# PolyU-IOR/HPR-LP-C

Hardware: AMD Instinct MI355X
Metric: HPR iterations/sec (FP64) (higher is better)
Workload: dtype f64

## Files before the change

hpr-lp-c_amd/csrc/kernels.hip:

```cpp
#include "kernels.h"
#include "group_table.h"
#include "values_body.h"

#include <algorithm>
#include <array>
#include <cstring>
#include <tuple>
#include <stdexcept>
#include <vector>
#include <cmath>
#include <type_traits>

namespace hprlp {

__device__ __forceinline__ double wave_sum(double v) {
#pragma unroll
    for (int off = 32; off > 0; off >>= 1) v += __shfl_xor(v, off, kWave);
    return v;
}

__device__ __forceinline__ double wave_max(double v) {
#pragma unroll
    for (int off = 32; off > 0; off >>= 1) v = fmax(v, __shfl_xor(v, off, kWave));
    return v;
// ... 199 lines not shown
                int j = rs;
                for (; j + 8 <= re; j += 8) {
#pragma unroll
                    for (int v = 0; v < NV; ++v) {
                        double p[8];
#pragma unroll
                        for (int u = 0; u < 8; ++u) p[u] = lds[wave][v][j + u];
#pragma unroll
                        for (int u = 0; u < 8; ++u) s[v] += p[u];
                    }
                }
                if (j < re) {
#pragma unroll
                    for (int v = 0; v < NV; ++v) {
                        double p[8];
#pragma unroll
                        for (int u = 0; u < 8; ++u) p[u] = lds[wave][v][min(j + u, re - 1)];
#pragma unroll
                        for (int u = 0; u < 8; ++u)
                            if (j + u < re) s[v] += p[u];
                    }
                }
                epi.apply(r0 + lane, rw, s, acc);
            }
        }
    }
    if constexpr (NACC > 0) block_store_partials_at<NACC, kWavesPerBlock, MaxAccs<Epi>::value>(acc, epi.partials, epi.stride, bid);
}

template <class Epi>
__global__ void __launch_bounds__(kThreads) k_spmv_fused(CsrDev A, Epi epi) {
    spmv_fused_body<Epi>(A, epi, blockIdx.x, gridDim.x);
}

__device__ __forceinline__ void lds_barrier() { asm volatile("s_waitcnt lgkmcnt(0)\n\ts_barrier" ::: "memory"); }

__device__ __forceinline__ int step_field(int a0, int a1, int a2, int a3, int r) {
    const int q = r >> 6;
    const int v = q == 0 ? a0 : (q == 1 ? a1 : (q == 2 ? a2 : a3));
    return __builtin_amdgcn_readlane(v, r & 63);
}

#ifndef HPRLP_PB_PHASE_STAMPS
#define HPRLP_PB_PHASE_STAMPS 0
#endif
#ifndef HPRLP_SWEEP_ED
#define HPRLP_SWEEP_ED 2
#define HPRLP_SWEEP_TD 1
#endif
#ifndef HPRLP_EPI_NT
#define HPRLP_EPI_NT 2
#endif

template <int ED, int TD, bool REP, bool STAMP = false, bool LOGTERM = false, int TC = kTileCols>
__device__ __forceinline__ void tiled_sweep(const TiledDev &t, int s0, int nst, int first, int count, const double *__restrict__ vec,
                                            int ncols, double *acc, double *ytile, int tid, unsigned long long *stamp = nullptr) {
    constexpr int NT = kTileThreads, R = kTileRows, K = kTileChunk;
    constexpr int TPT = TC / NT;
    static_assert(TC == kTileCols || TC == kTileColsNarrow, "tile width");
    typedef double d2_t __attribute__((ext_vector_type(2)));
    const int lane = tid & 63;
    auto sidx = [&](int i) { i = min(i, count - 1) + first; return s0 + (i < nst ? i : i - nst); };
    int seg = 0, lim = 0;
    int tc0 = 0, tc1 = 0, tc2 = 0, tc3 = 0, tb0 = 0, tb1 = 0, tb2 = 0, tb3 = 0, te0 = 0, te1 = 0, te2 = 0, te3 = 0;
    auto getstep = [&](int k, int &col0, int &eb, int &ee) {
        const int r = min(k, lim - 1) - seg;
        col0 = step_field(tc0, tc1, tc2, tc3, r);
        eb = step_field(tb0, tb1, tb2, tb3, r);
        ee = step_field(te0, te1, te2, te3, r);
    };
    struct Ent {
        d2_t va, vb;
        uint32_t i0, i1, i2;
    };
    typedef uint32_t u3_t __attribute__((ext_vector_type(3), aligned(4)));
    auto issue_entries = [&](Ent &E, int k) {
        int col0, eb, ee_;
        getstep(k, col0, eb, ee_);
        const int e = eb + K * tid;
        const int ee = (e < ee_) ? e : eb;
        E.va = __builtin_nontemporal_load(reinterpret_cast<const d2_t *>(t.tval + ee));
        E.vb = __builtin_nontemporal_load(reinterpret_cast<const d2_t *>(t.tval + ee) + 1);
        const u3_t w = __builtin_nontemporal_load(reinterpret_cast<const u3_t *>(t.tidx3 + (ee / K) * 3));
        E.i0 = w.x;
        E.i1 = w.y;
        E.i2 = w.z;
    };
    typedef double d2u_t __attribute__((ext_vector_type(2), aligned(8)));
    auto issue_tile = [&](double (&tl)[TPT], int k) {
        int col0, eb, ee_;
        getstep(k, col0, eb, ee_);
        static_assert(TPT % 2 == 0, "tile loads come in pairs");
#pragma unroll
        for (int j = 0; j < TPT / 2; ++j) {
            const int p = col0 + 2 * (tid + j * NT);
            const int q = min(p, ncols - 2);
            d2u_t v = *reinterpret_cast<const d2u_t *>(vec + q);
            if (q != p) v.x = v.y;
            tl[2 * j] = v.x;
            tl[2 * j + 1] = v.y;
        }
    };
    auto store_tile = [&](const double (&tl)[TPT]) {
#pragma unroll
        for (int j = 0; j < TPT / 2; ++j) {
            d2_t v;
            v.x = tl[2 * j];
            v.y = tl[2 * j + 1];
            reinterpret_cast<d2_t *>(ytile)[tid + j * NT] = v;
// ... 30 lines not shown
    auto same_tile = [&](int k) {
        if (k <= seg || k >= lim) return false;
        int c0, c1, eb, ee_;
        getstep(k, c0, eb, ee_);
        getstep(k - 1, c1, eb, ee_);
        return c0 == c1;
    };
    unsigned long long tq[6] = {0, 0, 0, 0, 0, 0}, ph[7] = {0, 0, 0, 0, 0, 0, 0};
    auto step = [&](Ent &E, double (&tl)[TPT], int k) {
        if (STAMP) tq[0] = __builtin_amdgcn_s_memtime();
        lds_barrier();
        if (STAMP) tq[1] = __builtin_amdgcn_s_memtime();
        if (STAMP) {
            store_tile(tl);
            tq[2] = __builtin_amdgcn_s_memtime();
            issue_tile(tl, k + TD);
            tq[3] = __builtin_amdgcn_s_memtime();
            lds_barrier();
            tq[4] = __builtin_amdgcn_s_memtime();
            process(E, k);
            asm volatile("s_waitcnt lgkmcnt(0)" ::: "memory");
            tq[5] = __builtin_amdgcn_s_memtime();
            issue_entries(E, k + ED);
            const unsigned long long t6 = __builtin_amdgcn_s_memtime();
            ph[0] += tq[1] - tq[0];
            ph[1] += tq[2] - tq[1];
            ph[2] += tq[3] - tq[2];
            ph[3] += tq[4] - tq[3];
            ph[4] += tq[5] - tq[4];
            ph[5] += t6 - tq[5];
            ph[6] += 1;
            return;
        }
        if (REP) {
            const bool keep = same_tile(k);
            if (!keep) {
                store_tile(tl);
            }
            if (!same_tile(k + TD)) issue_tile(tl, k + TD);
            if (!keep) lds_barrier();
        } else {
            store_tile(tl);
            issue_tile(tl, k + TD);
            lds_barrier();
        }
        process(E, k);
        issue_entries(E, k + ED);
    };
    for (seg = 0; seg < count; seg += 256) {
        lim = min(seg + 256, count);
        {
            const TileStep q0 = t.steps[sidx(seg + lane)], q1 = t.steps[sidx(seg + 64 + lane)];
            const TileStep q2 = t.steps[sidx(seg + 128 + lane)], q3 = t.steps[sidx(seg + 192 + lane)];
            tc0 = q0.col0; tb0 = q0.e_begin; te0 = q0.e_end;
            tc1 = q1.col0; tb1 = q1.e_begin; te1 = q1.e_end;
            tc2 = q2.col0; tb2 = q2.e_begin; te2 = q2.e_end;
            tc3 = q3.col0; tb3 = q3.e_begin; te3 = q3.e_end;
        }
        Ent E[ED];
        double tl[TD][TPT];
        __builtin_amdgcn_sched_barrier(0);
#pragma unroll
        for (int j = -(ED > TD ? ED : TD); j < 0; ++j) {
            if (j + TD >= 0) {
                issue_tile(tl[(j + TD) % TD], seg + j + TD);
                __builtin_amdgcn_sched_barrier(0);
            }
            if (j + ED >= 0) {
                issue_entries(E[(j + ED) % ED], seg + j + ED);
                __builtin_amdgcn_sched_barrier(0);
            }
        }
        constexpr int U = (ED * TD) % 2 == 0 && ED * TD > 2 ? ED * TD : 2 * ED * TD;
        static_assert(U % ED == 0 && U % TD == 0, "the unrolled body must return every register set to its role");
        bool done = false;
        for (int k = seg; !done;) {
#pragma unroll
            for (int u = 0; u < U; ++u) {
                step(E[u % ED], tl[u % TD], k);
                if (++k >= lim) {
                    done = true;
                    break;
                }
            }
        }
    }
    if (STAMP && tid == 0) {
#pragma unroll
        for (int i = 0; i < 7; ++i) stamp[i] += ph[i];
    }
}

template <int K>
__device__ __forceinline__ void remainder_steps(const TiledDev &t, int smid, int s1, double *acc, double *prod, double *bnd, int tid) {
    constexpr int NT = kTileThreads, NW = kTileThreads / 64;
    static_assert(K == 4 || K == 6 || K == 8, "code loads: one or two 16-byte loads, or two 12-byte loads, per lane");
    if (smid >= s1) return;
    const int wave = tid >> 6, lane = tid & 63;
    double *bnd_val = bnd;
    uint32_t *bnd_row = reinterpret_cast<uint32_t *>(bnd + NW);
    constexpr uint32_t NOROW = 0x10000u;
    double pv[K];
    uint32_t cv[K];
    TileStep st = t.steps[smid];
    auto issue = [&](const TileStep &z) {
        const int last = max(z.e_end - z.e_begin - 1, 0);
#pragma unroll
        for (int k = 0; k < K; ++k) pv[k] = __builtin_nontemporal_load(t.P + z.e_begin + min(tid + k * NT, last));
        const int c0 = min(K * tid, max(last + 1 - K, 0));
        if constexpr (K == 6) {
            typedef uint32_t u3_t __attribute__((ext_vector_type(3), aligned(4)));
            const u3_t w0 = __builtin_nontemporal_load(reinterpret_cast<const u3_t *>(t.rq + z.e_begin + c0));
            const u3_t w1 = __builtin_nontemporal_load(reinterpret_cast<const u3_t *>(t.rq + z.e_begin + c0 + 3));
            cv[0] = w0.x; cv[1] = w0.y; cv[2] = w0.z; cv[3] = w1.x; cv[4] = w1.y; cv[5] = w1.z;
        } else {
            typedef uint32_t u4_t __attribute__((ext_vector_type(4), aligned(4)));
            const u4_t w0 = __builtin_nontemporal_load(reinterpret_cast<const u4_t *>(t.rq + z.e_begin + c0));
            cv[0] = w0.x; cv[1] = w0.y; cv[2] = w0.z; cv[3] = w0.w;
            if constexpr (K == 8) {
                const u4_t w1 = __builtin_nontemporal_load(reinterpret_cast<const u4_t *>(t.rq + z.e_begin + c0 + 4));
                cv[4] = w1.x; cv[5] = w1.y; cv[6] = w1.z; cv[7] = w1.w;
            }
        }
    };
    issue(st);
    for (int s = smid; s < s1; ++s) {
        const int cnt = st.e_end - st.e_begin;
        const TileStep nxt = t.steps[min(s + 1, s1 - 1)];
        lds_barrier();
#pragma unroll
        for (int k = 0; k < K; ++k) {
            const int el = tid + k * NT;
            if (el < cnt) prod[el] = pv[k];
        }
        uint32_t code[K];
        {
            const int shift = K * tid - min(K * tid, max(cnt - K, 0));
#pragma unroll
            for (int u = 0; u < K; ++u) code[u] = cv[u];
            if (shift > 0 && shift < K) {
#pragma unroll
                for (int u = 0; u < K; ++u) {
                    uint32_t c = 0;
#pragma unroll
                    for (int q = 0; q < K; ++q) c = (q == u + shift) ? cv[q] : c;
                    code[u] = c;
                }
            }
        }
        if (s + 1 < s1) issue(nxt);
        lds_barrier();
        const int nv = min(max(cnt - K * tid, 0), K);
        uint32_t row[K];
        double pr[K];
#pragma unroll
        for (int u = 0; u < K; ++u) {
            const bool ok = u < nv;
// ... 21 lines not shown
        const bool open_in = lane > 0 && rf == rl_prev && rf != NOROW;
        double v = run;
        int f = (single && open_in) ? 0 : 1;
#pragma unroll
        for (int off = 1; off < 64; off <<= 1) {
            const double vu = __shfl_up(v, off, 64);
            const int fu = __shfl_up(f, off, 64);
            if (lane >= off && !f) {
                v += vu;
                f |= fu;
            }
        }
        const double v_prev = __shfl_up(v, 1, 64);
        const double carry = open_in ? v_prev : 0.0;
        const int next_open = __shfl_down(static_cast<int>(open_in), 1, 64);
        if (!single) acc[rf] += carry + head;
        const double tail = single ? carry + run : run;
        if (lane == 63) {
            bnd_row[wave] = rl;
            bnd_val[wave] = tail;
        } else if (!next_open && rl != NOROW) {
            acc[rl] += tail;
        }
        lds_barrier();
        if (tid < NW) {
            const uint32_t rw = bnd_row[tid];
            bool last_one = rw != NOROW;
            double tot = 0.0;
#pragma unroll
            for (int w = 0; w < NW; ++w) {
                const bool same = bnd_row[w] == rw;
                if (w <= tid && same) tot += bnd_val[w];
                if (w > tid && same) last_one = false;
            }
            if (last_one) acc[rw] += tot;
        }
        st = nxt;
    }
}

template <class Epi, class = void>
struct StagedLoads : std::false_type {};
template <class Epi>
struct StagedLoads<Epi, std::void_t<decltype(std::declval<const Epi &>().load_code(0))>> : std::true_type {};
template <class T>
__device__ __forceinline__ void needed_here(const T &v) {
    static_assert(sizeof(T) % sizeof(double) == 0 && alignof(T) == alignof(double), "a struct of doubles");
    double d[sizeof(T) / sizeof(double)];
    __builtin_memcpy(d, &v, sizeof(T));
#pragma unroll
    for (unsigned k = 0; k < sizeof(T) / sizeof(double); ++k) asm volatile("" ::"v"(d[k]));
}

template <class Epi, bool PUSH>
__device__ __forceinline__ void epilogue_rows(const Epi &epi, double *acc, double (&racc)[Epi::NACC > 0 ? Epi::NACC : 1], int r0, int nr, int tid) {
    constexpr int NT = kTileThreads, B = 4;
    if constexpr (StagedLoads<Epi>::value) {
        using Raw = decltype(epi.load_a(0));
        using Sel = decltype(epi.load_b(0, 0, 0u));
        auto issue_codes = [&](int b0, unsigned (&cd)[B]) {
#pragma unroll
            for (int u = 0; u < B; ++u) cd[u] = epi.load_code(r0 + min(b0 + tid + u * NT, nr - 1));
            __builtin_amdgcn_sched_barrier(0);
        };
        auto batch = [&](int b0, const unsigned (&cd)[B], unsigned (&cdn)[B]) {
            Raw ra[B];
            Sel rs[B];
            double sv[B][1];
#pragma unroll
            for (int u = 0; u < B; ++u) ra[u] = epi.load_a(r0 + min(b0 + tid + u * NT, nr - 1));
            __builtin_amdgcn_sched_barrier(0);
#pragma unroll
            for (int u = 0; u < B; ++u) rs[u] = epi.load_b(r0 + min(b0 + tid + u * NT, nr - 1), r0, cd[u]);
            __builtin_amdgcn_sched_barrier(0);
            issue_codes(b0 + B * NT, cdn);
#pragma unroll
            for (int u = 0; u < B; ++u) sv[u][0] = acc[min(b0 + tid + u * NT, nr - 1)];
#pragma unroll
            for (int u = 0; u < B; ++u) {
                needed_here(ra[u]);
                needed_here(rs[u]);
                asm volatile("" ::"v"(cdn[u]));
            }
            typename Epi::Row rw[B];
#pragma unroll
            for (int u = 0; u < B; ++u) rw[u] = epi.finish(cd[u], ra[u], rs[u]);
#pragma unroll
            for (int u = 0; u < B; ++u) {
                const int i = b0 + tid + u * NT;
                if (i < nr) {
                    if constexpr (PUSH) acc[i] = epi.apply(r0 + i, rw[u], sv[u], racc);
                    else epi.apply(r0 + i, rw[u], sv[u], racc);
                }
            }
        };
        if (nr <= 0) return;
        unsigned cd0[B], cd1[B];
        __builtin_amdgcn_sched_barrier(0);
        issue_codes(0, cd0);
#pragma unroll
        for (int u = 0; u < B; ++u) asm volatile("" ::"v"(cd0[u]));
        for (int b0 = 0;;) {
            batch(b0, cd0, cd1);
            if ((b0 += B * NT) >= nr) break;
            batch(b0, cd1, cd0);
            if ((b0 += B * NT) >= nr) break;
        }
    } else {
        for (int i0 = tid; i0 < nr; i0 += B * NT) {
            typename Epi::Row rw[B];
            double sv[B][1];
#pragma unroll
            for (int u = 0; u < B; ++u) {
                const int i = min(i0 + u * NT, nr - 1);
                rw[u] = epi.load_row(r0 + i);
                sv[u][0] = acc[i];
            }
#pragma unroll
            for (int u = 0; u < B; ++u) {
                const int i = i0 + u * NT;
                if (i < nr) {
                    if constexpr (PUSH) acc[i] = epi.apply(r0 + i, rw[u], sv[u], racc);
                    else epi.apply(r0 + i, rw[u], sv[u], racc);
                }
            }
        }
    }
}

__device__ __forceinline__ void push_products(const FarPush &f, const double *vals, int pb, int pe, int tid) {
    constexpr int NT = kTileThreads, U = 4;
    if (pb >= pe) return;
    double a4[U];
    int p4[U];
    uint16_t c4[U];
    auto load_batch = [&](int k0) {
#pragma unroll
        for (int u = 0; u < U; ++u) {
            const int z = min(k0 + u * NT, pe - 1);
            a4[u] = __builtin_nontemporal_load(f.val + z);
            p4[u] = __builtin_nontemporal_load(f.pos + z);
            c4[u] = __builtin_nontemporal_load(f.lcol + z);
        }
    };
    int k = pb + tid;
    load_batch(k);
    for (; k < pe; k += U * NT) {
        double prd[U];
        int ps[U];
#pragma unroll
        for (int u = 0; u < U; ++u) {
            prd[u] = a4[u] * vals[c4[u]];
// ... 11 lines not shown
    int lo = 0, hi = nr - 1;
    while (lo < hi) {
        const int mid = (lo + hi + 1) >> 1;
        if (tab_k[mid] <= k) lo = mid;
        else hi = mid - 1;
    }
    return tab_p[lo] + (k - tab_k[lo]);
}

__device__ __forceinline__ void push_products_runs(const FarPush &f, const double *vals, int *tab, int g, int pb, int pe, int tid) {
    constexpr int NT = kTileThreads, U = 4;
    if (pb >= pe) return;
    const int r0 = f.rptr[g], nr = f.rptr[g + 1] - r0;
    int *tab_k = tab, *tab_p = tab + kPbRunTabCap;
    double a4[U];
    uint16_t c4[U];
    auto load_batch = [&](int k0) {
#pragma unroll
        for (int u = 0; u < U; ++u) {
            const int z = min(k0 + u * NT, pe - 1);
            a4[u] = __builtin_nontemporal_load(f.val + z);
            c4[u] = __builtin_nontemporal_load(f.lcol + z);
        }
    };
    int k = pb + tid;
    load_batch(k);
    for (int i = tid; i < nr; i += NT) {
        tab_k[i] = f.rk[r0 + i];
        tab_p[i] = f.rp[r0 + i];
    }
    lds_barrier();
    int ps[U];
#pragma unroll
    for (int u = 0; u < U; ++u) ps[u] = run_position(tab_k, tab_p, nr, min(k + u * NT, pe - 1));
    for (; k < pe; k += U * NT) {
        double prd[U];
        int pc[U];
#pragma unroll
        for (int u = 0; u < U; ++u) {
            prd[u] = a4[u] * vals[c4[u]];
            pc[u] = ps[u];
        }
        const int kn = k + U * NT;
        if (kn < pe) load_batch(kn);
#pragma unroll
        for (int u = 0; u < U; ++u)
            if (k + u * NT < pe) f.P[pc[u]] = prd[u];
        if (kn < pe) {
#pragma unroll
            for (int u = 0; u < U; ++u) ps[u] = run_position(tab_k, tab_p, nr, min(kn + u * NT, pe - 1));
        }
    }
}

template <class Epi, bool REP, bool PUSH = false, bool NARROW = false>
__global__ void __launch_bounds__(kTileThreads, 4) k_tiled_fused(CsrDev A, Epi epi) {
    static_assert(Epi::NV == 1, "the tiled kernel stages one gathered vector");
    constexpr int NT = kTileThreads, RMAX = kTileRows, T = kTileCols;
    constexpr int NACC = Epi::NACC;
    __shared__ double acc[RMAX];
    __shared__ __attribute__((aligned(16))) double ytile[T];
    const TiledDev &t = A.tiled;
    const int tid = threadIdx.x;
    const int R = t.R;
    const int per = t.per, slots = gridDim.x / 8;
    const int slot = blockIdx.x / 8;
    double racc[NACC > 0 ? NACC : 1];
#pragma unroll
    for (int i = 0; i < (NACC > 0 ? NACC : 1); ++i) racc[i] = 0.0;
    epi.begin();
    int wg_round = 0;
    const bool wg_stamp = t.wgtimes && tid == 0 && (t.wg_filter == 0 || (PUSH && NACC == 0));
    if (wg_stamp) t.wgtimes[blockIdx.x * 8] = wall_clock64();
    for (int q = slot; q < per; q += slots) {
        const int sb = (blockIdx.x % 8) * per + q;
        if (sb >= t.nsb) break;
        const double *__restrict__ vec = epi.gv[0];
        lds_barrier();
        const int ncols = A.cols;
        for (int i = tid; i < R; i += NT) acc[i] = 0.0;
        const int s0 = t.sb_ptr[sb], smid = t.sb_mid[sb], s1 = t.sb_ptr[sb + 1];
        if (s0 < smid) tiled_sweep<HPRLP_SWEEP_ED, HPRLP_SWEEP_TD, REP, false, LogTerm<Epi>::value, NARROW ? kTileColsNarrow : kTileCols>(t, s0, smid - s0, t.steps[s0].rot, smid - s0, vec, ncols, acc, ytile, tid);
        remainder_steps<kTileRemK>(t, smid, s1, acc, ytile, ytile + kTileRemCap, tid);
        lds_barrier();
        const int r0 = sb * R;
        const int nr = min(R, A.rows - r0);
        int pb = 0, pe = 0;
        if constexpr (PUSH) {
            pb = epi.push.gptr[sb];
            pe = epi.push.gptr[sb + 1];
        }
        epilogue_rows<Epi, PUSH>(epi, acc, racc, r0, nr, tid);
        if constexpr (PUSH) {
            lds_barrier();
            push_products(epi.push, acc, pb, pe, tid);
        }
        if (wg_stamp && ++wg_round <= 5) t.wgtimes[blockIdx.x * 8 + wg_round] = wall_clock64();
    }
    if (wg_stamp) {
        t.wgtimes[blockIdx.x * 8 + 7] = wall_clock64();
        const unsigned hw = __builtin_amdgcn_s_getreg((31 << 11) | 4), xcc = __builtin_amdgcn_s_getreg((31 << 11) | 20);
        t.wgtimes[blockIdx.x * 8 + 6] = (static_cast<unsigned long long>(xcc & 0xfu) << 32) | hw;
    }
    if constexpr (NACC > 0) {
        __syncthreads();
        block_store_partials_in<NACC, kTileThreads / kWave, MaxAccs<Epi>::value>(racc, epi.partials, epi.stride, reinterpret_cast<double(*)[NACC]>(ytile));
    }
}

template <class Epi, bool PUSH = false>
__global__ void __launch_bounds__(kTileThreads, 4) k_pb_fused(CsrDev A, Epi epi) {
    static_assert(Epi::NV == 1, "one gathered vector");
    constexpr int NT = kTileThreads, K = kPbRemK, CAP = kPbRemCap, NW = kTileThreads / 64;
    constexpr int NACC = Epi::NACC;
    __shared__ double acc[kPbRowsMax];
    __shared__ __attribute__((aligned(16))) double prod[CAP];
    __shared__ double bnd[3 * NW];
    const TiledDev &t = A.tiled;
    const int tid = threadIdx.x;
    const int R = t.R;
    const int per = t.per, slots = gridDim.x / 8;
    const int slot = blockIdx.x / 8;
    double racc[NACC > 0 ? NACC : 1];
#pragma unroll
    for (int i = 0; i < (NACC > 0 ? NACC : 1); ++i) racc[i] = 0.0;
    epi.begin();
#if HPRLP_PB_PHASE_STAMPS
    unsigned long long ph[8] = {0, 0, 0, 0, 0, 0, 0, 0}, tq = wall_clock64(), tk0 = tq;
#define PB_STAMP(i) do { const unsigned long long now_ = wall_clock64(); ph[i] += now_ - tq; tq = now_; } while (0)
#else
#define PB_STAMP(i) do { } while (0)
#endif
    for (int q = slot; q < per; q += slots) {
        const int sb = (blockIdx.x % 8) * per + q;
        if (sb >= t.nsb) break;
        lds_barrier();
        for (int i = tid; i < R; i += NT) acc[i] = 0.0;
        const int smid = t.sb_mid[sb], s1 = t.sb_ptr[sb + 1];
        remainder_steps<K>(t, smid, s1, acc, prod, bnd, tid);
        lds_barrier();
        PB_STAMP(4);
        const int r0 = sb * R;
        const int nr = min(R, A.rows - r0);
        int pb = 0, pe = 0;
        if constexpr (PUSH) {
            pb = epi.push.gptr[sb];
            pe = epi.push.gptr[sb + 1];
        }
        epilogue_rows<Epi, PUSH>(epi, acc, racc, r0, nr, tid);
        PB_STAMP(5);
        if constexpr (PUSH) {
            lds_barrier();
            if (epi.push.rk) push_products_runs(epi.push, acc, reinterpret_cast<int *>(prod), sb, pb, pe, tid);
            else push_products(epi.push, acc, pb, pe, tid);
        }
        PB_STAMP(6);
    }
#if HPRLP_PB_PHASE_STAMPS
    if (t.wgtimes && tid == 0 && PUSH && NACC == 0) {
        ph[7] = wall_clock64() - tk0;
        for (int i = 0; i < 8; ++i) t.wgtimes[blockIdx.x * 8 + i] = ph[i];
    }
#endif
#undef PB_STAMP
    if constexpr (NACC > 0) {
        __syncthreads();
        block_store_partials_in<NACC, kTileThreads / kWave, MaxAccs<Epi>::value>(racc, epi.partials, epi.stride, reinterpret_cast<double(*)[NACC]>(prod));
    }
}

template <bool REP, bool STAMP = false, bool NARROW = false>
__global__ void __launch_bounds__(kTileThreads, 4) k_tiled_part(CsrDev A, const double *__restrict__ vec) {
    constexpr int NT = kTileThreads, RMAX = kTileRows, T = kTileCols;
    __shared__ double acc[RMAX];
    __shared__ __attribute__((aligned(16))) double ytile[T];
    const TiledDev &t = A.tiled;
    const int tid = threadIdx.x;
    const int R = t.R;
    const int per = (t.n_pieces + 7) / 8;
    const int pc = (blockIdx.x % 8) * per + blockIdx.x / 8;
    if (pc >= t.n_pieces) return;
    for (int sg = t.piece_ptr[pc]; sg < t.piece_ptr[pc + 1]; ++sg) {
        const int4 d = t.segs[sg];
        const int sb = d.x;
        lds_barrier();
        for (int i = tid; i < R; i += NT) acc[i] = 0.0;
        const int s0 = t.sb_ptr[sb], smid = t.sb_mid[sb], s1 = t.sb_ptr[sb + 1];
        unsigned long long *st = STAMP ? t.stamps + static_cast<size_t>(pc) * 16 : nullptr;
        unsigned long long c0 = 0, c1 = 0, c2 = 0;
        if (STAMP) c0 = __builtin_amdgcn_s_memtime();
        if (d.z > 0) tiled_sweep<3, 2, REP, STAMP, false, NARROW ? kTileColsNarrow : kTileCols>(t, s0, smid - s0, d.y, d.z, vec, A.cols, acc, ytile, tid, st);
        if (STAMP) c1 = __builtin_amdgcn_s_memtime();
        if (d.w) remainder_steps<kTileRemK>(t, smid, s1, acc, ytile, ytile + kTileRemCap, tid);
        lds_barrier();
        if (STAMP) c2 = __builtin_amdgcn_s_memtime();
        double *out = t.parts + static_cast<size_t>(sg) * R;
        for (int i = tid; i < R; i += NT) out[i] = acc[i];
        if (STAMP && tid == 0) {
            st[8] += c1 - c0;
            st[9] += c2 - c1;
            st[10] += __builtin_amdgcn_s_memtime() - c2;
        }
// ... 2502 lines not shown
```

hpr-lp-c_amd/csrc/tiled.cpp:

```cpp
#include "tiled.h"
#include "env.h"

#include <algorithm>
#include <cstdlib>
#include <cstring>
#include <string>
#include <thread>
#include <type_traits>

namespace hprlp {

namespace {

struct Local {
    std::vector<int> sb_steps, sb_mid;
    std::vector<TileStep> steps;
    std::vector<char> step_is_rem;
    std::vector<uint32_t> tidx;
    std::vector<int> tperm, rcol, rperm;
    std::vector<uint16_t> rrow;
    long dense = 0, pad = 0;
};

void build_range(int rows, int cols, const int *rp, const int *ci, int sb0, int sb1, Local *L, int R, int T, int rem_cap) {
// ... 292 lines not shown
    rcol.alloc_zero(h.n_rem + 8);
    rperm.alloc(h.n_rem + 8);
    rrow.alloc_zero(h.n_rem + 8);
    size_t to = 0, ro = 0;
    for (const TiledHost::Piece &pc : h.pieces) {
        if (!pc.tidx.empty()) {
            HIP_CHECK(hipMemcpy(tidx.p + to, pc.tidx.data(), pc.tidx.size() * sizeof(uint32_t), hipMemcpyHostToDevice));
            HIP_CHECK(hipMemcpy(tperm.p + to, pc.tperm.data(), pc.tperm.size() * sizeof(int), hipMemcpyHostToDevice));
        }
        if (!pc.rcol.empty()) {
            HIP_CHECK(hipMemcpy(rcol.p + ro, pc.rcol.data(), pc.rcol.size() * sizeof(int), hipMemcpyHostToDevice));
            HIP_CHECK(hipMemcpy(rperm.p + ro, pc.rperm.data(), pc.rperm.size() * sizeof(int), hipMemcpyHostToDevice));
            HIP_CHECK(hipMemcpy(rrow.p + ro, pc.rrow.data(), pc.rrow.size() * sizeof(uint16_t), hipMemcpyHostToDevice));
        }
        to += pc.tidx.size();
        ro += pc.rcol.size();
    }
    view.valid = true;
    view.R = R;
    view.T = T;
    view.rem_cap = rem_cap;
    view.nsb = nsb;
    view.sb_ptr = sb_ptr.p;
    view.sb_mid = sb_mid.p;
    view.steps = steps.p;
    view.tval = tval.p;
    pack_indices(nullptr);
    view.tidx3 = tidx3.p;
    finish_schedule(nullptr);
}

void DeviceTiled::compare_with(const TiledHost &h) const {
    auto fail = [](const std::string &what) { throw std::runtime_error("tiling check: " + what); };
    if (n_tile != static_cast<long>(h.n_tile)) fail("tile entries " + std::to_string(n_tile) + " vs " + std::to_string(h.n_tile));
    if (n_rem != static_cast<long>(h.n_rem)) fail("remainder entries " + std::to_string(n_rem) + " vs " + std::to_string(h.n_rem));
    if (dense_entries != h.dense_entries || padding != h.padding) fail("dense / padding totals");
    auto same = [&](const char *name, const auto &dbuf, const auto &host) {
        using T = typename std::decay<decltype(host[0])>::type;
        std::vector<T> dev(host.size());
        if (!host.empty()) HIP_CHECK(hipMemcpy(dev.data(), dbuf.p, host.size() * sizeof(T), hipMemcpyDeviceToHost));
        for (size_t i = 0; i < host.size(); ++i)
            if (std::memcmp(&dev[i], &host[i], sizeof(T)) != 0) fail(std::string(name) + " differs at " + std::to_string(i));
    };
    same("sb_ptr", sb_ptr, h.sb_ptr);
    same("sb_mid", sb_mid, h.sb_mid);
    if (static_cast<size_t>(n_steps) != h.steps.size()) fail("step count");
    {
        std::vector<TileStep> dev(h.steps.size());
        if (!dev.empty()) HIP_CHECK(hipMemcpy(dev.data(), steps.p, dev.size() * sizeof(TileStep), hipMemcpyDeviceToHost));
        for (size_t i = 0; i < dev.size(); ++i)
            if (dev[i].col0 != h.steps[i].col0 || dev[i].e_begin != h.steps[i].e_begin || dev[i].e_end != h.steps[i].e_end)
                fail("steps differ at " + std::to_string(i));
    }
    std::vector<uint32_t> a_tidx;
    std::vector<int> a_tperm, a_rcol, a_rperm;
    std::vector<uint16_t> a_rrow;
    for (const TiledHost::Piece &pc : h.pieces) {
        a_tidx.insert(a_tidx.end(), pc.tidx.begin(), pc.tidx.end());
        a_tperm.insert(a_tperm.end(), pc.tperm.begin(), pc.tperm.end());
        a_rcol.insert(a_rcol.end(), pc.rcol.begin(), pc.rcol.end());
        a_rperm.insert(a_rperm.end(), pc.rperm.begin(), pc.rperm.end());
        a_rrow.insert(a_rrow.end(), pc.rrow.begin(), pc.rrow.end());
    }
    {
        std::vector<uint32_t> packed(a_tidx.size() / 4 * 3);
        for (size_t c = 0; c < a_tidx.size() / 4; ++c) {
            const uint32_t e0 = a_tidx[4 * c], e1 = a_tidx[4 * c + 1], e2 = a_tidx[4 * c + 2], e3 = a_tidx[4 * c + 3];
            packed[3 * c] = e0 | (e1 << 24);
            packed[3 * c + 1] = (e1 >> 8) | (e2 << 16);
            packed[3 * c + 2] = (e2 >> 16) | (e3 << 8);
        }
        same("tidx3", tidx3, packed);
    }
    same("tperm", tperm, a_tperm);
    same("rcol", rcol, a_rcol);
    same("rperm", rperm, a_rperm);
    same("rrow", rrow, a_rrow);
}

}
```

hpr-lp-c_amd/csrc/tiled.h:

```cpp
#pragma once

#include <hip/hip_runtime.h>

#include <cstdint>
#include <vector>

#include "common.h"

namespace hprlp {

constexpr int kTileThreads = 512;
constexpr int kTileRows = 8192;
constexpr int kTileCols = 2048;
constexpr int kTileColsNarrow = 1024;
constexpr int kTileChunk = 4;
constexpr int kTileStepCap = kTileThreads * kTileChunk;
constexpr int kTileRemK = 4;
constexpr int kTileRemCap = (kTileThreads - 4) * kTileRemK;
constexpr int kTileRemRun = 16;
#ifndef HPRLP_PB_REM_K
#define HPRLP_PB_REM_K 8
#endif
constexpr int kPbRemK = HPRLP_PB_REM_K;
constexpr int kPbRemCap = kTileThreads * kPbRemK;
// ... 43 lines not shown
        return 0;
    }
};

#ifndef HPRLP_TILE_LAYERS
#define HPRLP_TILE_LAYERS 4
#endif
#ifndef HPRLP_TILE_LAYER_MIN
#define HPRLP_TILE_LAYER_MIN 1024
#endif
constexpr int kTileLayers = HPRLP_TILE_LAYERS;
constexpr int kTileLayerMin = HPRLP_TILE_LAYER_MIN;

constexpr int kTileResidentPerCu = 2;
constexpr int kFarGroup = kTileRows;
constexpr int kFarThreads = 512;
constexpr long kFarWorkMin = 32768;
constexpr long kFarWorkOverMean = 4;

struct TileStep {
    int col0;
    int e_begin;
    int e_end;
    int rot;
};

struct TiledDev {
    bool valid = false;
    int R = kTileRows;
    int rem_cap = kTileRemCap;
    int T = kTileCols;
    int G = kTileRows;
    int nsb = 0;
    int per = 0;
    int grid = 0;
    bool repeats = false;
    int n_pieces = 0;
    const int *piece_ptr = nullptr;
    const int4 *segs = nullptr;
    const int *slot_ptr = nullptr;
    double *parts = nullptr;
    const int4 *side_blk = nullptr;
    int side_nblk = 0;
    const int4 *side_long = nullptr;
    int side_nlong = 0;
    double *side_partial = nullptr;
    const int *side_rows = nullptr;
    double *base = nullptr;
    unsigned long long *stamps = nullptr;
    unsigned long long *wgtimes = nullptr;
    int wg_filter = 0;
    const int *sb_ptr = nullptr;
    const int *sb_mid = nullptr;
    const TileStep *steps = nullptr;
    const double *tval = nullptr;
    const uint32_t *tidx3 = nullptr;
    double *P = nullptr;
    const uint32_t *rq = nullptr;
    int n_groups = 0;
    const int *f_gptr = nullptr;
    const double *f_val = nullptr;
    const int *f_pos = nullptr;
    const uint16_t *f_lcol = nullptr;
    const int *f_rptr = nullptr;
    const int *f_rk = nullptr;
    const int *f_rp = nullptr;
    int f_maxruns = 0;
    const int4 *f_work = nullptr;
    int n_work = 0;
};

struct TiledHost {
    std::vector<int> sb_ptr, sb_mid;
    std::vector<TileStep> steps;
    struct Piece {
        std::vector<uint32_t> tidx;
        std::vector<int> tperm;
        std::vector<int> rcol, rperm;
        std::vector<uint16_t> rrow;
    };
    std::vector<Piece> pieces;
    size_t n_tile = 0, n_rem = 0;
    long dense_entries = 0;
    long padding = 0;
};

bool build_tiled(int rows, int cols, const int *rowptr, const int *col, TiledHost *out, int min_rows,
                 double min_dense_fraction, int R = kTileRows, int T = kTileCols, int rem_cap = kTileRemCap);

void tiled_host_check(int rows, int cols, const int *rp, const int *ci, int R, int T, double min_dense, long out[6]);

void compact_without_rows(long nnz, int rows, const int *rp_dev, const int *rp_c_dev, const int *col_dev, int *col_c, int *map_c, hipStream_t s);

struct DeviceTiled {
    DBuf<int> sb_ptr, sb_mid, tperm, rperm, rcol;
    DBuf<TileStep> steps;
    DBuf<uint32_t> tidx;
    DBuf<uint32_t> tidx3;
    DBuf<uint16_t> rrow;
    DBuf<double> tval;
    DBuf<double> P, f_val;
    DBuf<uint32_t> rq;
    DBuf<int> f_gptr, f_pos, f_perm;
    DBuf<int> f_rptr, f_rk, f_rp;
    DBuf<int4> f_work;
    DBuf<uint16_t> f_lcol;
    TiledDev view;
    long n_tile = 0, n_rem = 0;
    double rem_top_share = 0.0;
    long dense_entries = 0, padding = 0;
    int n_steps = 0;
    void upload(const TiledHost &h, int R = kTileRows, int T = kTileCols, int rem_cap = kTileRemCap);
    void pack_indices(hipStream_t s);
    void build_far(int cols, hipStream_t s, int G = kTileRows);
    void finish_schedule(hipStream_t s);
    int rot_period = 0;
    DBuf<double> parts;
    DBuf<int> piece_ptr, slot_ptr;
    DBuf<unsigned long long> stamps;
    void dump_stamps() const;
    DBuf<unsigned long long> wgtimes;
    DBuf<int4> side_blk, side_long;
    DBuf<int> side_rows;
    DBuf<double> side_partial, base;
    void set_side(int rows, const int *rowptr_host, const std::vector<int> &long_rows);
    void compose_perms(const int *map_dev, hipStream_t s);
    void dump_wgtimes() const;
    DBuf<int4> segs;
    bool build_on_device(int rows, int cols, long nnz, const int *rowptr, const int *col, int min_rows,
                         double min_dense_fraction, hipStream_t s, int R = kTileRows, int T = kTileCols, int rem_cap = kTileRemCap);
    void compare_with(const TiledHost &h) const;
};

void launch_tiled_refresh(const DeviceTiled &t, const double *csr_val, hipStream_t s);
void launch_tiled_refresh_log(const DeviceTiled &t, const double *csr_val, double *tval_log, double *fval_log, hipStream_t s);

}
```

hpr-lp-c_amd/csrc/tiled_build.hip:

```cpp
#include <algorithm>
#include <functional>
#include <cstdlib>
#include <hipcub/hipcub.hpp>

#include <vector>

#include "common.h"
#include "env.h"
#include "kernels.h"
#include "tiled.h"

namespace hprlp {

namespace {

constexpr int K = kTileChunk;
constexpr int kRowBits = kTileRowBits;

__device__ __forceinline__ int row_of_entry(const int *__restrict__ rowptr, int rows, int k) {
    int lo = 0, hi = rows;
    while (hi - lo > 1) {
        const int mid = lo + ((hi - lo) >> 1);
        if (rowptr[mid] <= k) lo = mid;
        else hi = mid;
// ... 285 lines not shown

__global__ void __launch_bounds__(kThreads) k_pack_codes(long nchunk, const uint32_t *__restrict__ code, uint32_t *__restrict__ packed) {
    const long c = static_cast<long>(blockIdx.x) * kThreads + threadIdx.x;
    if (c >= nchunk) return;
    const uint32_t e0 = code[4 * c], e1 = code[4 * c + 1], e2 = code[4 * c + 2], e3 = code[4 * c + 3];
    packed[3 * c] = e0 | (e1 << 24);
    packed[3 * c + 1] = (e1 >> 8) | (e2 << 16);
    packed[3 * c + 2] = (e2 >> 16) | (e3 << 8);
}

}

void DeviceTiled::pack_indices(hipStream_t s) {
    const long nchunk = n_tile / K;
    tidx3.alloc_zero(static_cast<size_t>(nchunk) * 3 + 8);
    if (nchunk > 0) hipLaunchKernelGGL(k_pack_codes, dim3(grid_for(nchunk)), dim3(kThreads), 0, s, nchunk, tidx.p, tidx3.p);
    HIP_CHECK(hipStreamSynchronize(s));
    tidx.release();
}

namespace {

__global__ void __launch_bounds__(kThreads) k_window_widths(int nsb, int T, const int *__restrict__ sb_ptr, const int *__restrict__ sb_mid,
                                                           const TileStep *__restrict__ steps, unsigned long long *__restrict__ out) {
    const int sb = blockIdx.x * kThreads + threadIdx.x;
    if (sb >= nsb) return;
    const int s0 = sb_ptr[sb], smid = sb_mid[sb];
    if (s0 >= smid) return;
    const int w = (steps[smid - 1].col0 - steps[s0].col0) / T + 1;
    atomicAdd(out, static_cast<unsigned long long>(w));
    atomicAdd(out + 1, 1ull);
    int rep = 0;
    for (int s = s0 + 1; s < smid; ++s) rep += steps[s].col0 == steps[s - 1].col0;
    if (rep) atomicAdd(out + 2, static_cast<unsigned long long>(rep));
}

__global__ void __launch_bounds__(kThreads) k_rotation(int nsb, int period, int T, const int *__restrict__ sb_ptr, const int *__restrict__ sb_mid,
                                                      TileStep *__restrict__ steps) {
    const int sb = blockIdx.x * kThreads + threadIdx.x;
    if (sb >= nsb) return;
    const int s0 = sb_ptr[sb], smid = sb_mid[sb];
    if (s0 >= smid) return;
    const int nst = smid - s0;
    const int w0 = steps[s0].col0 / T;
    const long target = static_cast<long>((w0 + period - 1) / period) * period * T;
    int lo = 0, hi = nst;
    while (lo < hi) {
        const int mid = (lo + hi) >> 1;
        if (steps[s0 + mid].col0 < target) lo = mid + 1; else hi = mid;
    }
    steps[s0].rot = lo < nst ? lo : 0;
}

}

void DeviceTiled::finish_schedule(hipStream_t s) {
    const int nsb = view.nsb;
    int dev = 0, cus = 256;
    HIP_CHECK(hipGetDevice(&dev));
    HIP_CHECK(hipDeviceGetAttribute(&cus, hipDeviceAttributeMultiprocessorCount, dev));
    const int resident = std::max(1, cus / 8) * kTileResidentPerCu;
    view.per = (nsb + 7) / 8;
    view.grid = 8 * std::min(view.per, resident);
    view.n_pieces = 0;
    int want = (nsb > 0 && nsb <= resident * 8) ? resident * 8 : 0;
    if (view.R < kTileRows && nsb >= cus) want = 0;
    if (view.rem_cap != kTileRemCap) want = 0;
    if (const char *e = env_get("HPRLP_TILE_PIECES")) want = std::max(0, std::atoi(e));
    if (want > 0 && nsb > 0) {
        std::vector<int> h_ptr(static_cast<size_t>(nsb) + 1), h_mid(static_cast<size_t>(nsb));
        sb_ptr.download(h_ptr.data(), h_ptr.size());
        sb_mid.download(h_mid.data(), h_mid.size());
        long total = 0;
        for (int sb = 0; sb < nsb; ++sb) total += h_ptr[sb + 1] - h_ptr[sb];
        const int np = static_cast<int>(std::max<long>(1, std::min<long>(want, std::max<long>(total, 1))));
        std::vector<int4> h_segs;
        std::vector<int> h_piece(static_cast<size_t>(np) + 1, 0), h_slot(static_cast<size_t>(nsb) + 1, 0);
        long g = 0;
        std::vector<std::vector<int4>> by_piece(static_cast<size_t>(np));
        for (int sb = 0; sb < nsb; ++sb) {
            const int nst = h_mid[sb] - h_ptr[sb];
            h_slot[sb] = 0;
            if (nst == 0) {
                const int pc = static_cast<int>(total > 0 ? std::min<long>(np - 1, g * np / total) : 0);
                by_piece[pc].push_back(make_int4(sb, 0, 0, 1));
                g += h_ptr[sb + 1] - h_mid[sb];
                continue;
            }
            int done = 0;
            while (done < nst) {
                const int pc = static_cast<int>(std::min<long>(np - 1, (g + done) * np / total));
                const long nxt = pc + 1 >= np ? total : ((static_cast<long>(pc) + 1) * total + np - 1) / np;
                const int cnt = static_cast<int>(std::min<long>(nst - done, std::max<long>(1, nxt - (g + done))));
                by_piece[pc].push_back(make_int4(sb, done, cnt, done + cnt == nst ? 1 : 0));
                done += cnt;
            }
            g += h_ptr[sb + 1] - h_ptr[sb];
        }
        for (int pc = 0; pc < np; ++pc) {
            h_piece[pc] = static_cast<int>(h_segs.size());
            for (const int4 &sg : by_piece[pc]) h_segs.push_back(sg);
        }
        h_piece[np] = static_cast<int>(h_segs.size());
        {
            size_t i = 0;
            for (int sb = 0; sb < nsb; ++sb) {
                h_slot[sb] = static_cast<int>(i);
                while (i < h_segs.size() && h_segs[i].x == sb) ++i;
            }
            h_slot[nsb] = static_cast<int>(i);
            if (i != h_segs.size()) throw std::runtime_error("piece schedule: segments out of super-block order");
        }
        piece_ptr.alloc(h_piece.size()); piece_ptr.upload(h_piece.data(), h_piece.size());
        slot_ptr.alloc(h_slot.size()); slot_ptr.upload(h_slot.data(), h_slot.size());
        segs.alloc(h_segs.size()); segs.upload(h_segs.data(), h_segs.size());
        parts.alloc_zero(h_segs.size() * static_cast<size_t>(view.R));
        view.n_pieces = np;
        view.piece_ptr = piece_ptr.p;
        view.slot_ptr = slot_ptr.p;
        view.segs = segs.p;
        view.parts = parts.p;
        if (const char *e = env_get("HPRLP_TILE_STAMPS"); e && e[0] == '1' && !view.repeats) {
            stamps.alloc_zero(static_cast<size_t>(np) * 16);
            view.stamps = stamps.p;
        }
    }
    if (const char *e = env_get("HPRLP_WG_TIMES"); e && (e[0] == '1' || e[0] == '2') && view.grid > 0) {
        wgtimes.alloc_zero(static_cast<size_t>(view.grid) * 8);
        view.wgtimes = wgtimes.p;
        view.wg_filter = e[0] == '2';
    }
    rot_period = 0;
    if (nsb <= 0 || n_steps <= 0) return;
    {
        DBuf<unsigned long long> acc(3);
        HIP_CHECK(hipMemsetAsync(acc.p, 0, 3 * sizeof(unsigned long long), s));
        hipLaunchKernelGGL(k_window_widths, dim3(grid_for(nsb)), dim3(kThreads), 0, s, nsb, view.T, sb_ptr.p, sb_mid.p, steps.p, acc.p);
        unsigned long long h[3] = {0, 0, 0};
        HIP_CHECK(hipMemcpyAsync(h, acc.p, sizeof(h), hipMemcpyDeviceToHost, s));
        HIP_CHECK(hipStreamSynchronize(s));
        if (h[1] > 0) rot_period = static_cast<int>((h[0] + h[1] - 1) / h[1]);
        view.repeats = h[2] > 0;
    }
    if (const char *e = env_get("HPRLP_TILE_ROT")) rot_period = std::atoi(e);
    if (rot_period > 0) hipLaunchKernelGGL(k_rotation, dim3(grid_for(nsb)), dim3(kThreads), 0, s, nsb, rot_period, view.T, sb_ptr.p, sb_mid.p, steps.p);
    HIP_CHECK(hipStreamSynchronize(s));
}

bool DeviceTiled::build_on_device(int rows, int cols, long nnz, const int *rowptr, const int *col, int min_rows,
                                  double min_dense_fraction, hipStream_t s, int R, int T, int rem_cap) {
    if (rem_cap != kTileRemCap && rem_cap != kPbRemCap) throw std::runtime_error("tiled build: unsupported remainder step size");
    if (rem_cap == kPbRemCap && R > kPbRowsMax) throw std::runtime_error("tiled build: the all-remainder form takes super-blocks of at most 4096 rows");
    if (rows < min_rows || rows <= 0 || cols <= 0 || nnz <= 0 || nnz >= 2000000000L) return false;
    if (R < 64 || R > kTileRows || R % 64 != 0) throw std::runtime_error("tiled build: unsupported super-block height");
    if (T != kTileCols && T != kTileColsNarrow) throw std::runtime_error("tiled build: unsupported tile width");
    const int nsb = (rows + R - 1) / R;
    const int ntile = (cols + T - 1) / T;
    int tile_bits = 1;
    while ((1 << tile_bits) < ntile) ++tile_bits;
    int sb_bits = 1;
    while ((1 << sb_bits) < nsb) ++sb_bits;
    const int key_bits = sb_bits + tile_bits + kRowBits;

    DBuf<unsigned long long> key_in(static_cast<size_t>(nnz)), skey(static_cast<size_t>(nnz));
    DBuf<int> idx_in(static_cast<size_t>(nnz)), sperm(static_cast<size_t>(nnz));
    hipLaunchKernelGGL(k_make_keys, dim3(grid_for(nnz)), dim3(kThreads), 0, s, nnz, rows, tile_bits, R, T, rowptr, col, key_in.p, idx_in.p);
    size_t tmp_bytes = 0;
    HIP_CHECK(hipcub::DeviceRadixSort::SortPairs(nullptr, tmp_bytes, key_in.p, skey.p, idx_in.p, sperm.p, static_cast<int>(nnz), kRowBits,
                                                 key_bits, s));
    {
        DBuf<char> tmp(tmp_bytes + 16);
        HIP_CHECK(hipcub::DeviceRadixSort::SortPairs(tmp.p, tmp_bytes, key_in.p, skey.p, idx_in.p, sperm.p, static_cast<int>(nnz), kRowBits,
                                                     key_bits, s));
        HIP_CHECK(hipStreamSynchronize(s));
    }
    key_in.release();
    idx_in.release();

    DBuf<int> head(static_cast<size_t>(nnz)), run_incl(static_cast<size_t>(nnz));
    hipLaunchKernelGGL(k_run_heads, dim3(grid_for(nnz)), dim3(kThreads), 0, s, nnz, skey.p, head.p);
    HIP_CHECK(hipcub::DeviceScan::InclusiveSum(nullptr, tmp_bytes, head.p, run_incl.p, static_cast<int>(nnz), s));
    {
        DBuf<char> tmp(tmp_bytes + 16);
        HIP_CHECK(hipcub::DeviceScan::InclusiveSum(tmp.p, tmp_bytes, head.p, run_incl.p, static_cast<int>(nnz), s));
        HIP_CHECK(hipStreamSynchronize(s));
    }
    int nruns = 0;
    HIP_CHECK(hipMemcpy(&nruns, run_incl.p + (nnz - 1), sizeof(int), hipMemcpyDeviceToHost));
    DBuf<int> run_start(static_cast<size_t>(nruns) + 1);
    hipLaunchKernelGGL(k_run_starts, dim3(grid_for(nnz)), dim3(kThreads), 0, s, nnz, head.p, run_incl.p, run_start.p);
    {
        const int end = static_cast<int>(nnz);
        HIP_CHECK(hipMemcpyAsync(run_start.p + nruns, &end, sizeof(int), hipMemcpyHostToDevice, s));
        HIP_CHECK(hipStreamSynchronize(s));
    }
    head.release();
    run_incl.release();

// ... 531 lines not shown
```

Before: 790.0.

## Prefetch next super-block descriptor and epilogue codes to hide load latency

Packs per-super-block start, mid, end and rotation into one int4 descriptor table built at setup, so the next super-block's descriptor and push ranges are fetched while the current sweep runs. It also hoists the first remainder step's bounds and the epilogue's first code loads ahead of the remainder phase. The aim is to remove serialized dependent global loads between phases of the fused SpMV kernel. The cost is extra registers held across the sweep, which could reduce occupancy, plus one more small setup kernel.

```diff
diff --git a/hpr-lp-c_amd/csrc/kernels.hip b/hpr-lp-c_amd/csrc/kernels.hip
--- a/hpr-lp-c_amd/csrc/kernels.hip
+++ b/hpr-lp-c_amd/csrc/kernels.hip
@@ -275,9 +275,13 @@
 #define HPRLP_EPI_NT 2
 #endif
 
-template <int ED, int TD, bool REP, bool STAMP = false, bool LOGTERM = false, int TC = kTileCols>
+struct NoHook {
+    __device__ __forceinline__ void operator()() const {}
+};
+template <int ED, int TD, bool REP, bool STAMP = false, bool LOGTERM = false, int TC = kTileCols, class After = NoHook>
 __device__ __forceinline__ void tiled_sweep(const TiledDev &t, int s0, int nst, int first, int count, const double *__restrict__ vec,
-                                            int ncols, double *acc, double *ytile, int tid, unsigned long long *stamp = nullptr) {
+                                            int ncols, double *acc, double *ytile, int tid, unsigned long long *stamp = nullptr,
+                                            After after_table = After()) {
     constexpr int NT = kTileThreads, R = kTileRows, K = kTileChunk;
     constexpr int TPT = TC / NT;
     static_assert(TC == kTileCols || TC == kTileColsNarrow, "tile width");
@@ -414,6 +418,7 @@
         {
             const TileStep q0 = t.steps[sidx(seg + lane)], q1 = t.steps[sidx(seg + 64 + lane)];
             const TileStep q2 = t.steps[sidx(seg + 128 + lane)], q3 = t.steps[sidx(seg + 192 + lane)];
+            after_table();
             tc0 = q0.col0; tb0 = q0.e_begin; te0 = q0.e_end;
             tc1 = q1.col0; tb1 = q1.e_begin; te1 = q1.e_end;
             tc2 = q2.col0; tb2 = q2.e_begin; te2 = q2.e_end;
@@ -453,8 +458,9 @@
     }
 }
 
-template <int K>
-__device__ __forceinline__ void remainder_steps(const TiledDev &t, int smid, int s1, double *acc, double *prod, double *bnd, int tid) {
+template <int K, class After = NoHook>
+__device__ __forceinline__ void remainder_steps(const TiledDev &t, int smid, int s1, double *acc, double *prod, double *bnd, int tid,
+                                                After after_first = After(), const TileStep *first = nullptr) {
     constexpr int NT = kTileThreads, NW = kTileThreads / 64;
     static_assert(K == 4 || K == 6 || K == 8, "code loads: one or two 16-byte loads, or two 12-byte loads, per lane");
     if (smid >= s1) return;
@@ -464,7 +470,13 @@
     constexpr uint32_t NOROW = 0x10000u;
     double pv[K];
     uint32_t cv[K];
-    TileStep st = t.steps[smid];
+    TileStep st;
+    if (first) {
+        st = *first;
+    } else {
+        st = t.steps[smid];
+        after_first();
+    }
     auto issue = [&](const TileStep &z) {
         const int last = max(z.e_end - z.e_begin - 1, 0);
 #pragma unroll
@@ -592,9 +604,27 @@
     for (unsigned k = 0; k < sizeof(T) / sizeof(double); ++k) asm volatile("" ::"v"(d[k]));
 }
 
+constexpr int kEpiBatch = 4;
+template <class Epi>
+struct WithBase;
+template <class Epi>
+struct EarlyCodes : std::true_type {};
+template <class Epi>
+struct EarlyCodes<WithBase<Epi>> : std::false_type {};
+template <class Epi>
+__device__ __forceinline__ void epilogue_first_codes(const Epi &epi, int r0, int nr, int tid, unsigned (&cd)[kEpiBatch]) {
+    if constexpr (StagedLoads<Epi>::value) {
+        __builtin_amdgcn_sched_barrier(0);
+#pragma unroll
+        for (int u = 0; u < kEpiBatch; ++u) cd[u] = epi.load_code(r0 + min(tid + u * kTileThreads, nr - 1));
+        __builtin_amdgcn_sched_barrier(0);
+    }
+}
+
 template <class Epi, bool PUSH>
-__device__ __forceinline__ void epilogue_rows(const Epi &epi, double *acc, double (&racc)[Epi::NACC > 0 ? Epi::NACC : 1], int r0, int nr, int tid) {
-    constexpr int NT = kTileThreads, B = 4;
+__device__ __forceinline__ void epilogue_rows(const Epi &epi, double *acc, double (&racc)[Epi::NACC > 0 ? Epi::NACC : 1], int r0, int nr, int tid,
+                                              unsigned (&cd0)[kEpiBatch]) {
+    constexpr int NT = kTileThreads, B = kEpiBatch;
     if constexpr (StagedLoads<Epi>::value) {
         using Raw = decltype(epi.load_a(0));
         using Sel = decltype(epi.load_b(0, 0, 0u));
@@ -634,10 +664,10 @@
                 }
             }
         };
-        if (nr <= 0) return;
-        unsigned cd0[B], cd1[B];
+        if constexpr (PUSH) __builtin_assume(nr > 0);
+        else if (nr <= 0) return;
+        unsigned cd1[B];
         __builtin_amdgcn_sched_barrier(0);
-        issue_codes(0, cd0);
 #pragma unroll
         for (int u = 0; u < B; ++u) asm volatile("" ::"v"(cd0[u]));
         for (int b0 = 0;;) {
@@ -755,6 +785,27 @@
         }
     }
 }
+
+template <bool PUSH>
+struct SbLook {
+    int s0, smid, s1, rot, pb, pe;
+    template <class Epi>
+    __device__ __forceinline__ void fetch(const TiledDev &t, const Epi &epi, int sb) {
+        const int4 d = t.sb_desc[sb];
+        int b = 0, e = 0;
+        if constexpr (PUSH) {
+            const int g = min(sb, t.nsb - 1);
+            b = epi.push.gptr[g];
+            e = epi.push.gptr[g + 1];
+        }
+        s0 = __builtin_amdgcn_readfirstlane(d.x);
+        smid = __builtin_amdgcn_readfirstlane(d.y);
+        s1 = __builtin_amdgcn_readfirstlane(d.z);
+        rot = __builtin_amdgcn_readfirstlane(d.w);
+        pb = __builtin_amdgcn_readfirstlane(b);
+        pe = __builtin_amdgcn_readfirstlane(e);
+    }
+};
 
 template <class Epi, bool REP, bool PUSH = false, bool NARROW = false>
 __global__ void __launch_bounds__(kTileThreads, 4) k_tiled_fused(CsrDev A, Epi epi) {
@@ -775,25 +826,35 @@
     int wg_round = 0;
     const bool wg_stamp = t.wgtimes && tid == 0 && (t.wg_filter == 0 || (PUSH && NACC == 0));
     if (wg_stamp) t.wgtimes[blockIdx.x * 8] = wall_clock64();
+    const int sb_first = (blockIdx.x % 8) * per;
+    SbLook<PUSH> look;
+    look.fetch(t, epi, sb_first + min(slot, per - 1));
     for (int q = slot; q < per; q += slots) {
-        const int sb = (blockIdx.x % 8) * per + q;
+        const int sb = sb_first + q;
         if (sb >= t.nsb) break;
         const double *__restrict__ vec = epi.gv[0];
         lds_barrier();
         const int ncols = A.cols;
         for (int i = tid; i < R; i += NT) acc[i] = 0.0;
-        const int s0 = t.sb_ptr[sb], smid = t.sb_mid[sb], s1 = t.sb_ptr[sb + 1];
-        if (s0 < smid) tiled_sweep<HPRLP_SWEEP_ED, HPRLP_SWEEP_TD, REP, false, LogTerm<Epi>::value, NARROW ? kTileColsNarrow : kTileCols>(t, s0, smid - s0, t.steps[s0].rot, smid - s0, vec, ncols, acc, ytile, tid);
-        remainder_steps<kTileRemK>(t, smid, s1, acc, ytile, ytile + kTileRemCap, tid);
-        lds_barrier();
+        const int s0 = look.s0, smid = look.smid, s1 = look.s1, rot = look.rot, pb = look.pb, pe = look.pe;
+        TileStep rem0 = {0, 0, 0, 0};
+        auto look_ahead = [&]() {
+            int2 r = make_int2(0, 0);
+            if (smid < s1) r = make_int2(t.steps[smid].e_begin, t.steps[smid].e_end);
+            look.fetch(t, epi, sb_first + min(q + slots, per - 1));
+            rem0.e_begin = __builtin_amdgcn_readfirstlane(r.x);
+            rem0.e_end = __builtin_amdgcn_readfirstlane(r.y);
+        };
+        if (s0 < smid) tiled_sweep<HPRLP_SWEEP_ED, HPRLP_SWEEP_TD, REP, false, LogTerm<Epi>::value, NARROW ? kTileColsNarrow : kTileCols>(t, s0, smid - s0, rot, smid - s0, vec, ncols, acc, ytile, tid, nullptr, look_ahead);
+        else look_ahead();
         const int r0 = sb * R;
         const int nr = min(R, A.rows - r0);
-        int pb = 0, pe = 0;
-        if constexpr (PUSH) {
-            pb = epi.push.gptr[sb];
-            pe = epi.push.gptr[sb + 1];
-        }
-        epilogue_rows<Epi, PUSH>(epi, acc, racc, r0, nr, tid);
+        unsigned cd0[kEpiBatch];
+        if constexpr (EarlyCodes<Epi>::value) epilogue_first_codes(epi, r0, nr, tid, cd0);
+        remainder_steps<kTileRemK>(t, smid, s1, acc, ytile, ytile + kTileRemCap, tid, NoHook(), &rem0);
+        lds_barrier();
+        if constexpr (!EarlyCodes<Epi>::value) epilogue_first_codes(epi, r0, nr, tid, cd0);
+        epilogue_rows<Epi, PUSH>(epi, acc, racc, r0, nr, tid, cd0);
         if constexpr (PUSH) {
             lds_barrier();
             push_products(epi.push, acc, pb, pe, tid);
@@ -834,23 +895,26 @@
 #else
 #define PB_STAMP(i) do { } while (0)
 #endif
+    const int sb_first = (blockIdx.x % 8) * per;
+    SbLook<PUSH> look;
+    look.fetch(t, epi, sb_first + min(slot, per - 1));
     for (int q = slot; q < per; q += slots) {
-        const int sb = (blockIdx.x % 8) * per + q;
+        const int sb = sb_first + q;
         if (sb >= t.nsb) break;
         lds_barrier();
         for (int i = tid; i < R; i += NT) acc[i] = 0.0;
-        const int smid = t.sb_mid[sb], s1 = t.sb_ptr[sb + 1];
-        remainder_steps<K>(t, smid, s1, acc, prod, bnd, tid);
+        const int smid = look.smid, s1 = look.s1, pb = look.pb, pe = look.pe;
+        auto look_ahead = [&]() { look.fetch(t, epi, sb_first + min(q + slots, per - 1)); };
+        const int r0 = sb * R;
+        const int nr = min(R, A.rows - r0);
+        unsigned cd0[kEpiBatch];
+        if constexpr (EarlyCodes<Epi>::value) epilogue_first_codes(epi, r0, nr, tid, cd0);
+        if (smid < s1) remainder_steps<K>(t, smid, s1, acc, prod, bnd, tid, look_ahead);
+        else look_ahead();
         lds_barrier();
         PB_STAMP(4);
-        const int r0 = sb * R;
-        const int nr = min(R, A.rows - r0);
-        int pb = 0, pe = 0;
-        if constexpr (PUSH) {
-            pb = epi.push.gptr[sb];
-            pe = epi.push.gptr[sb + 1];
-        }
-        epilogue_rows<Epi, PUSH>(epi, acc, racc, r0, nr, tid);
+        if constexpr (!EarlyCodes<Epi>::value) epilogue_first_codes(epi, r0, nr, tid, cd0);
+        epilogue_rows<Epi, PUSH>(epi, acc, racc, r0, nr, tid, cd0);
         PB_STAMP(5);
         if constexpr (PUSH) {
             lds_barrier();
diff --git a/hpr-lp-c_amd/csrc/tiled.cpp b/hpr-lp-c_amd/csrc/tiled.cpp
--- a/hpr-lp-c_amd/csrc/tiled.cpp
+++ b/hpr-lp-c_amd/csrc/tiled.cpp
@@ -368,6 +368,21 @@
             if (dev[i].col0 != h.steps[i].col0 || dev[i].e_begin != h.steps[i].e_begin || dev[i].e_end != h.steps[i].e_end)
                 fail("steps differ at " + std::to_string(i));
     }
+    {
+        std::vector<int4> dev(static_cast<size_t>(8) * std::max(view.per, 1));
+        if (sb_desc.n != dev.size()) fail("sb_desc length");
+        sb_desc.download(dev.data(), dev.size());
+        std::vector<TileStep> st(h.steps.size());
+        if (!st.empty()) HIP_CHECK(hipMemcpy(st.data(), steps.p, st.size() * sizeof(TileStep), hipMemcpyDeviceToHost));
+        for (size_t sb = 0; sb < dev.size(); ++sb) {
+            int4 want = make_int4(0, 0, 0, 0);
+            if (sb < h.sb_mid.size()) {
+                want = make_int4(h.sb_ptr[sb], h.sb_mid[sb], h.sb_ptr[sb + 1], 0);
+                if (want.x < want.y) want.w = st[want.x].rot;
+            }
+            if (dev[sb].x != want.x || dev[sb].y != want.y || dev[sb].z != want.z || dev[sb].w != want.w) fail("sb_desc differs at " + std::to_string(sb));
+        }
+    }
     std::vector<uint32_t> a_tidx;
     std::vector<int> a_tperm, a_rcol, a_rperm;
     std::vector<uint16_t> a_rrow;
diff --git a/hpr-lp-c_amd/csrc/tiled.h b/hpr-lp-c_amd/csrc/tiled.h
--- a/hpr-lp-c_amd/csrc/tiled.h
+++ b/hpr-lp-c_amd/csrc/tiled.h
@@ -119,6 +119,7 @@
     int wg_filter = 0;
     const int *sb_ptr = nullptr;
     const int *sb_mid = nullptr;
+    const int4 *sb_desc = nullptr;
     const TileStep *steps = nullptr;
     const double *tval = nullptr;
     const uint32_t *tidx3 = nullptr;
@@ -162,6 +163,7 @@
 struct DeviceTiled {
     DBuf<int> sb_ptr, sb_mid, tperm, rperm, rcol;
     DBuf<TileStep> steps;
+    DBuf<int4> sb_desc;
     DBuf<uint32_t> tidx;
     DBuf<uint32_t> tidx3;
     DBuf<uint16_t> rrow;
diff --git a/hpr-lp-c_amd/csrc/tiled_build.hip b/hpr-lp-c_amd/csrc/tiled_build.hip
--- a/hpr-lp-c_amd/csrc/tiled_build.hip
+++ b/hpr-lp-c_amd/csrc/tiled_build.hip
@@ -361,6 +361,14 @@
     steps[s0].rot = lo < nst ? lo : 0;
 }
 
+__global__ void __launch_bounds__(kThreads) k_sb_desc(int nsb, const int *__restrict__ sb_ptr, const int *__restrict__ sb_mid,
+                                                     const TileStep *__restrict__ steps, int4 *__restrict__ desc) {
+    const int sb = blockIdx.x * kThreads + threadIdx.x;
+    if (sb >= nsb) return;
+    const int s0 = sb_ptr[sb], smid = sb_mid[sb], s1 = sb_ptr[sb + 1];
+    desc[sb] = make_int4(s0, smid, s1, s0 < smid ? steps[s0].rot : 0);
+}
+
 }
 
 void DeviceTiled::finish_schedule(hipStream_t s) {
@@ -371,6 +379,8 @@
     const int resident = std::max(1, cus / 8) * kTileResidentPerCu;
     view.per = (nsb + 7) / 8;
     view.grid = 8 * std::min(view.per, resident);
+    sb_desc.alloc_zero(static_cast<size_t>(8) * std::max(view.per, 1));
+    view.sb_desc = sb_desc.p;
     view.n_pieces = 0;
     int want = (nsb > 0 && nsb <= resident * 8) ? resident * 8 : 0;
     if (view.R < kTileRows && nsb >= cus) want = 0;
@@ -453,6 +463,7 @@
     }
     if (const char *e = env_get("HPRLP_TILE_ROT")) rot_period = std::atoi(e);
     if (rot_period > 0) hipLaunchKernelGGL(k_rotation, dim3(grid_for(nsb)), dim3(kThreads), 0, s, nsb, rot_period, view.T, sb_ptr.p, sb_mid.p, steps.p);
+    hipLaunchKernelGGL(k_sb_desc, dim3(grid_for(nsb)), dim3(kThreads), 0, s, nsb, sb_ptr.p, sb_mid.p, steps.p, sb_desc.p);
     HIP_CHECK(hipStreamSynchronize(s));
 }
 
```

Result: no change. 785.0 (-0.6%).
